# zhoubin-me/agent0

Measured on NVIDIA B200. Metric: replay_sample_target_transitions_per_sec, higher is better.
Workload: dtype u8 frames / f32 targets / f64 n-step returns

## Files before the change

### agent0_b200/_lib.py

```python
import ctypes as C
import os

import torch

_PKG = os.path.dirname(os.path.abspath(__file__))
LIB_PATH = os.environ.get("A0_LIB") or os.path.join(_PKG, "libagent0_b200.so")

A0_SLOTS = 8
A0_REC_META_I32 = 14
A0_MAX_NSTEP = 16
A0_MAX_ACTIONS = 32
A0_MAX_QUANTILES = 256
PTR_FRAMES, PTR_REC_SLOTS, PTR_REC_INFO, PTR_TREE, PTR_MAX_P = range(5)
OPT_PDL = 1
K2B_PLAN_MAX = 1024
K2B_PLAN_BYTES = 90176


def lz4_stride(frame_bytes):
    n = 8 * int(frame_bytes)
    return (n + n // 255 + 20 + 15) // 16 * 16

_vp, _i32, _i64, _f32, _f64 = C.c_void_p, C.c_int32, C.c_int64, C.c_float, C.c_double


class LossCommon(C.Structure):
    _fields_ = [("B", _i32), ("A", _i32), ("action", _vp), ("reward", _vp), ("done", _vp),
                ("weight", _vp), ("gamma_n", _f32), ("alpha", _f32), ("eps", _f32),
                ("loss", _vp), ("prio", _vp), ("max_p", _vp)]


class Plan(C.Structure):
    _fields_ = [("m", _i32), ("n_new", _i32), ("n_marks", _i32), ("new_frame_pos", C.POINTER(_i32)),
                ("rec_meta", C.POINTER(_i32)), ("marks", C.POINTER(_i32))]


class Merge(C.Structure):
    _fields_ = [("n_place", _i64), ("place", C.POINTER(_i64)), ("n_rec", _i64), ("record_map", C.POINTER(_i64)),
                ("n_tail", _i64), ("tails", C.POINTER(_i64)), ("stride_hint", _i64)]


IX_HEAD_Q, IX_TAIL_Q, IX_HEAD_FS, IX_TOP, IX_REC_CAPACITY, IX_FRAME_CAPACITY, IX_NSTEP, IX_AGE_LIMIT, \
    IX_MAX_CHUNK, IX_STATE_WORDS = range(10)
INGEST_FRAMES_ON_DEVICE, INGEST_FRAMES_PINNED, INGEST_COPY_STREAM = 1, 2, 4

SIGNATURES = {
    "a0_version": (_i32, []),
    "a0_last_error": (C.c_char_p, []),
    "a0_set_option": (_i32, [_i32, _i64]),
    "a0_get_option": (_i32, [_i32, C.POINTER(C.c_int64)]),
    "a0_rb_create": (_i32, [C.POINTER(_vp), _i64, _i64, _i32, _i32]),
    "a0_rb_destroy": (_i32, [_vp]),
    "a0_rb_reset": (_i32, [_vp, _vp]),
    "a0_rb_ptr": (_vp, [_vp, _i32]),
    "a0_rb_tree_leaves": (_i64, [_vp]),
    "a0_ix_create": (_i32, [C.POINTER(_vp), _i64, _i64, _i32, _i64]),
    "a0_ix_destroy": (_i32, [_vp]),
    "a0_ix_state": (_i32, [_vp, _vp]),
    "a0_ix_sampleable": (_vp, [_vp]),
    "a0_ix_set_stack": (_i32, [_vp, _i64, _vp]),
    "a0_ix_get_stack": (_i32, [_vp, _i64, _vp]),
    "a0_ix_resolve_shift": (_i32, [_vp, _vp, _vp, _i32, _vp]),
    "a0_ix_plan": (_i32, [_vp, _vp, _vp, _i32, _i32, _vp, _vp, _vp, C.POINTER(Plan)]),
    "a0_dd_create": (_i32, [C.POINTER(_vp), _i32]),
    "a0_dd_destroy": (_i32, [_vp]),
    "a0_dd_resolve": (_i32, [_vp, _vp, _vp, _vp, _i32, _vp, _vp, C.POINTER(_i32)]),
    "a0_ex_create": (_i32, [C.POINTER(_vp), _vp, _vp]),
    "a0_ex_destroy": (_i32, [_vp]),
    "a0_ex_extend": (_i32, [_vp, _vp, _vp, _vp, _vp, _vp, _vp, _i32, _f32, _vp]),
    "a0_ex_extend_v": (_i32, [_vp, _vp, _vp, _vp, _vp, _vp, _vp, _i32, _f32, _vp]),
    "a0_ex_decode": (_i32, [_vp, _vp, _vp, _i32, _vp, _vp, _vp]),
    "a0_ex_resolve": (_i32, [_vp, _vp, _vp, _i32, _vp, _vp, C.POINTER(_i32)]),
    "a0_ex_last_timing": (_i32, [_vp, _vp]),
    "a0_lz4_encode": (_i32, [_vp, _i32, _i32, _vp, _vp, _vp, _vp]),
    "a0_ix_serialize": (_i32, [_vp, _vp, _i64, C.POINTER(_i64)]),
    "a0_ix_deserialize": (_i32, [_vp, _vp, _i64]),
    "a0_ckpt_save": (_i32, [_vp, _vp, _vp, C.c_char_p, _vp, _i64, _vp]),
    "a0_ckpt_load": (_i32, [_vp, _vp, _vp, C.c_char_p, _vp, _i64, C.POINTER(_i64), _vp]),
    "a0_ckpt_last_timing": (_i32, [_vp]),
    "a0_ix_merge": (_i32, [_vp, _i32, _vp, _vp, _vp, _vp, _vp, _vp, _vp, _vp, _vp, _vp, _vp, C.POINTER(Merge)]),
    "a0_ckpt_info": (_i32, [C.c_char_p, _vp, _vp, _i64]),
    "a0_ckpt_merge": (_i32, [_vp, _vp, _vp, _vp, _i32, _vp, _vp, _vp, _vp, _i64, _vp, _vp]),
    "a0_rb_ingest_plan": (_i32, [_vp, C.POINTER(Plan), _vp, _vp, _i32, _f32, _vp]),
    "a0_rb_ingest_steps": (_i32, [_vp, _vp, _vp, _vp, _vp, _i32, _vp, _vp, _vp, _i32, _f32, _vp]),
    "a0_rb_ingest_steps_dyn": (_i32, [_vp, _vp, _vp, _vp, _vp, _i32, _vp, _vp, _vp, _i32, _f32, _f32, _i32, _vp]),
    "a0_rb_append": (_i32, [_vp, _vp, _vp, _i32, _vp, _i32, _vp]),
    "a0_pt_mark": (_i32, [_vp, _vp, _i32, _f32, _vp]),
    "a0_pt_update": (_i32, [_vp, _vp, _vp, _i32, _f32, _f32, _vp]),
    "a0_pt_update_report": (_i32, [_vp, _vp, _vp, _i32, _f32, _f32, _vp, _vp, _vp]),
    "a0_pt_update_overlapped": (_i32, [_vp, _vp, _vp, _i32, _f32, _f32, _vp, _vp, _vp]),
    "a0_pt_update_plan": (_i32, [_vp, _vp, _i32, _vp, _vp]),
    "a0_pt_update_apply": (_i32, [_vp, _vp, _vp, _i32, _f32, _f32, _vp, _vp, _vp, _vp]),
    "a0_host_map": (_i32, [_vp, C.POINTER(_vp)]),
    "a0_pt_set": (_i32, [_vp, _vp, _vp, _i32, _vp]),
    "a0_rb_set_dynamic": (_i32, [_vp, _f32, _f32, _f32, _vp]),
    "a0_pt_sample": (_i32, [_vp, _vp, _i32, _i32, _f32, _f32, _f32, _i32, _vp, _vp, _vp, _vp]),
    "a0_pt_sample_rng": (_i32, [_vp, C.c_uint64, _i64, _i32, _i32, _f32, _f32, _f32, _i32, _vp, _vp, _vp, _vp, _vp]),
    "a0_pt_rng_seek": (_i32, [_vp, C.c_uint64, _vp]),
    "a0_pt_sample_unique": (_i32, [_vp, C.c_uint64, _i64, _i32, _i32, _f32, _f32, _f32, _i32, _vp, _vp, _vp, _vp, _vp]),
    "a0_rb_gather": (_i32, [_vp, _vp, _i32, _i32, _f64, _vp, _vp, _vp, _vp, _vp, _vp, _vp, _i32, _vp]),
    "a0_rb_sample_gather": (_i32, [_vp, _vp, C.c_uint64, _i64, _i32, _i32, _f32, _f32, _f32, _i32, _vp, _vp, _vp, _i32, _f64,
                                   _vp, _vp, _vp, _vp, _vp, _vp, _vp, _vp]),
    "a0_rb_sample_mail": (_i32, [_vp, _vp, C.c_uint64, _i64, _i32, _i32, _f32, _f32, _f32, _i32, _vp, _vp, _vp, _vp]),
    "a0_rb_gather_mail": (_i32, [_vp, _i32, _i32, _i32, _i32, _f64, _vp, _vp, _vp, _vp, _vp, _vp, _vp, _vp]),
    "a0_rb_gather_unpaired": (_i32, [_vp, _i32, _vp, _vp]),
    "a0_rb_check_fault": (_i32, [_vp]),
    "a0_rb_gather_f32": (_i32, [_vp, _vp, _i32, _i32, _f64, _vp, _vp, _i32, _vp, _vp, _vp, _vp, _vp, _vp, _vp]),
    "a0_rb_gather_bf16": (_i32, [_vp, _vp, _i32, _i32, _f64, _vp, _vp, _i32, _vp, _vp, _vp, _vp, _vp, _vp, _vp]),
    "a0_loss_dqn": (_i32, [C.POINTER(LossCommon), _vp, _vp, _vp, _vp, _vp]),
    "a0_loss_mdqn": (_i32, [C.POINTER(LossCommon), _vp, _vp, _vp, _f32, _f32, _vp, _vp]),
    "a0_loss_c51": (_i32, [C.POINTER(LossCommon), _vp, _vp, _vp, _vp, _i32, _f32, _f32, _vp, _vp, _vp]),
    "a0_c51_div_check": (_i32, [_f32, _f32, _i32, _vp, _vp]),
    "a0_loss_quantile": (_i32, [C.POINTER(LossCommon), _i32, _vp, _vp, _vp, _vp, _i32, _i32, _vp,
                                _vp, _vp, _vp, _vp, _vp]),
    "a0_act_epsilon_greedy": (_i32, [_vp, _i32, _i32, _f64, _vp, _vp, _vp, _vp, _vp, _vp, _vp]),
    "a0_u8_to_f32": (_i32, [_vp, _vp, _i64, _i32, _vp]),
}

_lib = None


def load():
    global _lib
    if _lib is not None:
        return _lib
    if not os.path.exists(LIB_PATH):
        raise RuntimeError(
            f"{LIB_PATH} is missing: build it with `python -m agent0_b200.build` "
            "(agent0_b200 has no CPU fallback)")
    lib = C.CDLL(LIB_PATH)
    for name, (res, args) in SIGNATURES.items():
        fn = getattr(lib, name)
        fn.restype, fn.argtypes = res, args
    _lib = lib
    return lib


_pyingest = False


def pyingest():
    global _pyingest
    if _pyingest is False:
        path = os.path.join(_PKG, "_a0_pyingest.so")
        _pyingest = None
        if os.path.exists(path):
            try:
                h = C.PyDLL(path)
                h.a0_py_unpack.restype = _i64
                h.a0_py_unpack.argtypes = [C.py_object, _i64, _vp, _vp, _vp, _vp, _vp, _vp]
                h.a0_py_release.restype = None
                h.a0_py_release.argtypes = [_i64, _vp]
                h.a0_py_buffer_size.restype = _i64
                _pyingest = h
            except OSError:
                _pyingest = None
    return _pyingest


def check(rc, what):
    if rc != 0:
        msg = load().a0_last_error().decode(errors="replace")
        raise RuntimeError(f"{what} failed (code {rc}): {msg}")

# ... 61 lines not shown
```

### agent0_b200/csrc/a0_targets.cu

```cuda
#include <stdlib.h>

#include "a0_common.cuh"
#ifdef A0_TRACE
A0_TRACE_SETTER(a0_trace_set_targets)
#endif

struct A0Common {
  int32_t B, A;
  const int64_t* action;
  const float* reward;
  const float* done;
  const float* weight;
  float gamma_n, alpha, eps;
  float* loss;
  float* prio;
  float* max_p;
};

static inline A0Common a0_unpack(const a0_loss_common_t* c) {
  A0Common k;
  k.B = c->B; k.A = c->A; k.action = c->action; k.reward = c->reward; k.done = c->done;
  k.weight = c->weight; k.gamma_n = c->gamma_n; k.alpha = c->alpha; k.eps = c->eps;
  k.loss = c->loss; k.prio = c->prio; k.max_p = c->max_p;
  return k;
// ... 292 lines not shown
#pragma unroll
  for (int k = 0; k < C51_MAXR; ++k) m[k] = s_m[wid][lane + 32 * k];

  A0_TX(4);
  const float lse = logf(ose);
  float ce = 0.0f, msum = 0.0f;
#pragma unroll
  for (int k = 0; k < C51_MAXR; ++k)
    if (k < R && lane + 32 * k < M) { ce += m[k] * ((l[k] - omx) - lse); msum += m[k]; }
  ce = a0_warp_sum(ce);
  msum = a0_warp_sum(msum);
  A0_TX(5);
  float* grow = grad + (size_t)b * A * M;
  for (int a2 = 0; a2 < A; ++a2) {
    if (a2 == a) continue;
    for (int j = lane; j < M; j += 32) grow[(size_t)a2 * M + j] = 0.0f;
  }
#pragma unroll
  for (int k = 0; k < C51_MAXR; ++k) {
    const int j = lane + 32 * k;
    if (k < R && j < M) {
      const float sm = expf((l[k] - omx) - lse);
      grow[(size_t)a * M + j] = w * (sm * msum - m[k]);
      if (target_prob) target_prob[(size_t)b * M + j] = m[k];
    }
  }
  A0_TX(6);
  if (lane == 0) a0_emit(c, b, -ce);
  A0_TX(7);
#ifdef A0_TRACE
  _t2 = _t2 * 0 + (unsigned long long)_c0;
#endif
  if (threadIdx.x == 0) A0_TEND(4);
}


__device__ __forceinline__ float a0_warp_max_redux(float v) {
  float m;
  asm("redux.sync.max.f32 %0, %1, 0xffffffff;" : "=f"(m) : "f"(v));
  return m;
}

__device__ __forceinline__ float a0_c51_div_delta(float nu, float delta, double rdelta) {
  const double q0 = __dmul_rn((double)nu, rdelta);
  const double rem = __fma_rn(-q0, (double)delta, (double)nu);
  return __double2float_rn(__fma_rn(rem, rdelta, q0));
}

static void a0_c51_delta(float vmin, float vmax, int32_t M, float* delta, double* rdelta) {
  *delta = (vmax - vmin) / (float)(M - 1);
  *rdelta = 1.0 / (double)*delta;
}

template <int WARPS>
__global__ void __launch_bounds__(WARPS * 32)
a0_k4_c51_fast(const A0Common c, const float* __restrict__ logits, const float* __restrict__ tgt_logits,
               const float* __restrict__ qsel, const float* __restrict__ atoms, int32_t M, float vmin, float vmax,
               float delta, double rdelta, float* __restrict__ grad, float* __restrict__ target_prob) {
  __shared__ float s_t[WARPS][4][72];
  A0_T0();
  A0_PDL_PROLOGUE();
  A0_TMID();
#ifdef A0_TRACE
  const long long _c0 = clock64();
#endif
  const int lane = threadIdx.x & 31;
  const int wid = threadIdx.x >> 5;
  const int b = blockIdx.x * WARPS + wid;
  if (b >= c.B) return;
  const int A = c.A;
  const bool in0 = lane < M, in1 = lane + 32 < M;
  float lo_all[C51_SPEC_A][2], tg_all[C51_SPEC_A][2], qs[C51_SPEC_A];
  const float* lrow = logits + (size_t)b * A * M + lane;
  const float* trow = tgt_logits + (size_t)b * A * M + lane;
  const float* qrow = qsel + (size_t)b * A;
#pragma unroll
  for (int a2 = 0; a2 < C51_SPEC_A; ++a2) {
    const bool on = a2 < A;
    lo_all[a2][0] = (on && in0) ? lrow[a2 * M] : -INFINITY;
    lo_all[a2][1] = (on && in1) ? lrow[a2 * M + 32] : -INFINITY;
    tg_all[a2][0] = (on && in0) ? trow[a2 * M] : -INFINITY;
    tg_all[a2][1] = (on && in1) ? trow[a2 * M + 32] : -INFINITY;
    qs[a2] = on ? qrow[a2] : -INFINITY;
  }
  const int a = (int)c.action[b];
  const float r = c.reward[b], d = c.done[b], w = c.weight[b];
  const float z0 = in0 ? atoms[lane] : 0.0f, z1 = in1 ? atoms[lane + 32] : 0.0f;
  float(*terms)[72] = s_t[wid];
#pragma unroll
  for (int t = 0; t < 4; ++t) {
    terms[t][lane] = 0.0f;
    terms[t][lane + 32] = 0.0f;
  }
  const int AM = A * M, r0 = a * M;
  float* gb = grad + (size_t)b * AM;
  for (int e = lane; e < AM; e += 32)
    if (e < r0 || e >= r0 + M) gb[e] = 0.0f;
  int a_star = 0;
  float best = qs[0];
#pragma unroll
  for (int a2 = 1; a2 < C51_SPEC_A; ++a2)
    if (qs[a2] > best) { best = qs[a2]; a_star = a2; }
  float l0 = -INFINITY, l1 = -INFINITY, p0 = -INFINITY, p1 = -INFINITY;
#pragma unroll
  for (int a2 = 0; a2 < C51_SPEC_A; ++a2) {
    if (a2 == a) { l0 = lo_all[a2][0]; l1 = lo_all[a2][1]; }
    if (a2 == a_star) { p0 = tg_all[a2][0]; p1 = tg_all[a2][1]; }
  }
  A0_TX(0);
  const float omx = a0_warp_max_redux(fmaxf(l0, l1)), mx = a0_warp_max_redux(fmaxf(p0, p1));
  A0_TX(1);
  const float eo0 = expf(in0 ? l0 - omx : -INFINITY), eo1 = expf(in1 ? l1 - omx : -INFINITY);
  p0 = expf(in0 ? p0 - mx : -INFINITY);
  p1 = expf(in1 ? p1 - mx : -INFINITY);
  float ose = eo0 + eo1, se = p0 + p1;
  const float gm = __fmul_rn(c.gamma_n, __fsub_rn(1.0f, d));
  const float tz0 = fminf(fmaxf(__fadd_rn(r, __fmul_rn(gm, z0)), vmin), vmax);
  const float tz1 = fminf(fmaxf(__fadd_rn(r, __fmul_rn(gm, z1)), vmin), vmax);
  const float bs0 = a0_c51_div_delta(__fsub_rn(tz0, vmin), delta, rdelta);
  const float bs1 = a0_c51_div_delta(__fsub_rn(tz1, vmin), delta, rdelta);
  const int c0 = max((int)ceilf(bs0) - 1, 0), c1 = max((int)ceilf(bs1) - 1, 0);
  const int k0 = in0 ? c0 : -1, k1 = in1 ? c1 : -1;
  const float fl0 = __fsub_rn((float)(c0 + 1), bs0), fu0 = __fsub_rn(bs0, (float)c0);
  const float fl1 = __fsub_rn((float)(c1 + 1), bs1), fu1 = __fsub_rn(bs1, (float)c1);
  unsigned join0 = 0, join1 = 0;
#pragma unroll
  for (int s = 0; s < 5; ++s) {
    const int q0 = __shfl_up_sync(0xffffffffu, k0, 1 << s), q1 = __shfl_up_sync(0xffffffffu, k1, 1 << s);
    if (lane >= (1 << s) && q0 == k0) join0 |= 1u << s;
    if (lane >= (1 << s) && q1 == k1) join1 |= 1u << s;
  }
  const int n0 = __shfl_down_sync(0xffffffffu, k0, 1), n1 = __shfl_down_sync(0xffffffffu, k1, 1);
  const bool tail0 = k0 >= 0 && (lane == 31 || n0 != k0), tail1 = k1 >= 0 && (lane == 31 || n1 != k1);
#pragma unroll
  for (int o = 16; o > 0; o >>= 1) {
    const float a_ = __shfl_xor_sync(0xffffffffu, ose, o);
    const float b_ = __shfl_xor_sync(0xffffffffu, se, o);
    ose += a_;
    se += b_;
  }
  const float lse = logf(ose);
  const float ls0 = (l0 - omx) - lse, ls1 = (l1 - omx) - lse;
  float sm0 = expf(ls0), sm1 = expf(ls1);
  A0_TX(2);
  float wl0 = 0.0f, wu0 = 0.0f, wl1 = 0.0f, wu1 = 0.0f;
  {
    const float q0 = __fdiv_rn(p0 != 0.0f ? p0 : 1.0f, se), q1 = __fdiv_rn(p1 != 0.0f ? p1 : 1.0f, se);
    const float pj0 = p0 != 0.0f ? q0 : 0.0f, pj1 = p1 != 0.0f ? q1 : 0.0f;
    if (in0) { wl0 = __fmul_rn(pj0, fl0); wu0 = __fmul_rn(pj0, fu0); }
    if (in1) { wl1 = __fmul_rn(pj1, fl1); wu1 = __fmul_rn(pj1, fu1); }
  }
  A0_TX(3);
#pragma unroll
  for (int s = 0; s < 5; ++s) {
    const float a0_ = __shfl_up_sync(0xffffffffu, wl0, 1 << s), b0_ = __shfl_up_sync(0xffffffffu, wu0, 1 << s);
    const float a1_ = __shfl_up_sync(0xffffffffu, wl1, 1 << s), b1_ = __shfl_up_sync(0xffffffffu, wu1, 1 << s);
    if (join0 >> s & 1u) { wl0 = __fadd_rn(wl0, a0_); wu0 = __fadd_rn(wu0, b0_); }
    if (join1 >> s & 1u) { wl1 = __fadd_rn(wl1, a1_); wu1 = __fadd_rn(wu1, b1_); }
  }
  asm volatile("" : "+f"(sm0), "+f"(sm1));
  __syncwarp();
  if (tail0) { terms[0][k0] = wl0; terms[2][k0 + 1] = wu0; }
  if (tail1) { terms[1][k1] = wl1; terms[3][k1 + 1] = wu1; }
  __syncwarp();
  const float m0 = __fadd_rn(__fadd_rn(__fadd_rn(terms[0][lane], terms[1][lane]), terms[2][lane]), terms[3][lane]);
  const float m1 = __fadd_rn(__fadd_rn(__fadd_rn(terms[0][lane + 32], terms[1][lane + 32]), terms[2][lane + 32]),
                             terms[3][lane + 32]);
  A0_TX(4);
  float ce = 0.0f, msum = 0.0f;
  if (in0) { ce += m0 * ls0; msum += m0; }
  if (in1) { ce += m1 * ls1; msum += m1; }
#pragma unroll
  for (int o = 16; o > 0; o >>= 1) {
    const float a_ = __shfl_xor_sync(0xffffffffu, ce, o);
    const float b_ = __shfl_xor_sync(0xffffffffu, msum, o);
    ce += a_;
    msum += b_;
  }
  A0_TX(5);
  if (lane == 0) a0_emit(c, b, -ce);
  const float g0 = w * (sm0 * msum - m0), g1 = w * (sm1 * msum - m1);
  if (in0) gb[r0 + lane] = g0;
  if (in1) gb[r0 + lane + 32] = g1;
  if (target_prob) {
    if (in0) target_prob[(size_t)b * M + lane] = m0;
    if (in1) target_prob[(size_t)b * M + lane + 32] = m1;
  }
  A0_TX(6);
  A0_TX(7);
#ifdef A0_TRACE
  _t2 = _t2 * 0 + (unsigned long long)_c0;
#endif
  if (threadIdx.x == 0) A0_TEND(4);
}

static int g_c51_fast = -1;
static bool a0_option_c51_fast() {
  if (g_c51_fast < 0) {
    const char* e = getenv("A0_C51_FAST");
    g_c51_fast = e ? (atoi(e) != 0) : 1;
  }
  return g_c51_fast != 0;
}
void a0_set_c51_fast(int on) { g_c51_fast = on != 0; }

extern "C" int a0_loss_c51(const a0_loss_common_t* c, const float* logits, const float* tgt_logits,
                           const float* qsel, const float* atoms, int32_t M, float vmin, float vmax, float* grad,
                           float* target_prob, a0_stream_t stream) {
  int rc = a0_check_common(c, "a0_loss_c51");
  if (rc) return rc;
  A0_REQUIRE(logits && tgt_logits && atoms && grad, "a0_loss_c51: NULL tensor");
  A0_REQUIRE(M >= 2 && M <= C51_MAXR * 32, "a0_loss_c51: num_atoms %d outside [2,%d]", M, C51_MAXR * 32);
  A0_REQUIRE(vmax > vmin, "a0_loss_c51: vmax must exceed vmin");
  if (c->B == 0) return A0_OK;
  float delta;
  double rdelta;
  a0_c51_delta(vmin, vmax, M, &delta, &rdelta);
  if (qsel && c->A <= C51_SPEC_A && M <= 64 && delta > 0.0f && delta < INFINITY && a0_option_c51_fast()) {
    static int warps = 0;
    if (!warps) {
      const char* e = getenv("A0_C51_WARPS");
      warps = e ? atoi(e) : C51_FAST_WARPS;
      if (warps != 1 && warps != 2 && warps != 4 && warps != 8 && warps != 16 && warps != 32) warps = C51_FAST_WARPS;
    }
    const unsigned grid = (unsigned)((c->B + warps - 1) / warps);
#define A0_C51_FAST_LAUNCH(W)                                                                                              \
    A0_LAUNCH(a0_k4_c51_fast<W>, grid, W * 32, 0, (cudaStream_t)stream, 1, A0_PDL_K4, a0_unpack(c), logits, tgt_logits, qsel,   \
              atoms, M, vmin, vmax, delta, rdelta, grad, target_prob)
    if (warps == 1) A0_C51_FAST_LAUNCH(1);
    else if (warps == 2) A0_C51_FAST_LAUNCH(2);
    else if (warps == 4) A0_C51_FAST_LAUNCH(4);
    else if (warps == 8) A0_C51_FAST_LAUNCH(8);
    else if (warps == 16) A0_C51_FAST_LAUNCH(16);
    else A0_C51_FAST_LAUNCH(32);
#undef A0_C51_FAST_LAUNCH
    return A0_OK;
  }
  A0_LAUNCH(a0_k4_c51, (unsigned)((c->B + C51_WARPS - 1) / C51_WARPS), C51_WARPS * 32, 0, (cudaStream_t)stream, 1, A0_PDL_K4,
            a0_unpack(c), logits, tgt_logits, qsel, atoms, M, vmin, vmax, grad, target_prob);
  return A0_OK;
}

__global__ void a0_c51_div_check_kernel(uint32_t hi, float delta, double rdelta, unsigned long long* out) {
  unsigned long long bad = 0, first = ~0ull;
  for (unsigned long long u = blockIdx.x * (unsigned long long)blockDim.x + threadIdx.x; u <= hi;
       u += (unsigned long long)gridDim.x * blockDim.x) {
    const float nu = __uint_as_float((uint32_t)u);
    if (__float_as_uint(a0_c51_div_delta(nu, delta, rdelta)) != __float_as_uint(__fdiv_rn(nu, delta))) {
      ++bad;
      first = min(first, u);
    }
  }
  if (bad) {
    atomicAdd(out, bad);
    atomicMin(out + 1, first);
  }
}

extern "C" int a0_c51_div_check(float vmin, float vmax, int32_t M, unsigned long long* out, a0_stream_t stream) {
  A0_REQUIRE(out != nullptr, "a0_c51_div_check: NULL output");
  A0_REQUIRE(M >= 2 && vmax > vmin, "a0_c51_div_check: M %d, vmin %g, vmax %g", M, (double)vmin, (double)vmax);
  float delta;
  double rdelta;
  a0_c51_delta(vmin, vmax, M, &delta, &rdelta);
  A0_REQUIRE(delta > 0.0f && delta < INFINITY, "a0_c51_div_check: delta %g is zero or infinite", (double)delta);
  const float hi = vmax - vmin;
  A0_REQUIRE(hi < INFINITY, "a0_c51_div_check: vmax - vmin overflows");
  uint32_t hb;
  memcpy(&hb, &hi, sizeof(hb));
  a0_c51_div_check_kernel<<<148 * 8, 256, 0, (cudaStream_t)stream>>>(hb, delta, rdelta, out);
  A0_LAUNCH_CHECK();
  return A0_OK;
}

constexpr int QH_SPEC_A = 8;

__device__ __forceinline__ float a0_block_sum(float v, float* red, int nwarps) {
  v = a0_warp_sum(v);
  __syncthreads();
  if ((threadIdx.x & 31) == 0) red[threadIdx.x >> 5] = v;
  __syncthreads();
  float s = 0.0f;
  for (int i = 0; i < nwarps; ++i) s += red[i];
  return s;
}

template <bool SPEC>
__global__ void __launch_bounds__(A0_MAX_QUANTILES)
a0_k4_quantile(const A0Common c, int32_t layout, const float* __restrict__ q, const float* __restrict__ qt,
               const float* __restrict__ taus, const float* __restrict__ qsel, int32_t Ni, int32_t Nj,
               float* __restrict__ grad, const float* __restrict__ q_bar, const float* __restrict__ taus_full,
               float* __restrict__ fraction_loss, float* __restrict__ grad_taus) {
  __shared__ float sT[A0_MAX_QUANTILES];
// ... 592 lines not shown
```

### agent0_b200/hotloop.py

```python
from __future__ import annotations

import ctypes as C

import numpy as np
import torch

from . import _lib

ALGOS = ("dqn", "mdqn", "c51", "qr", "iqn", "fqf")


def wave_plan(L, B, frame_bytes, spec="auto"):
    if not spec or L < 2:
        return None
    if isinstance(spec, str):
        assert spec == "auto", spec
        if B * 16 * frame_bytes >= 10_000_000:
            sizes = [1] * L
        else:
            sizes, w = [1], 1
            while sum(sizes) < L:
                sizes.append(min(w, L - sum(sizes)))
                w *= 2
            if len(sizes) > 1 and sizes[-1] < sizes[-2]:
                tail = sizes.pop()
                sizes[-1] += tail
    else:
        sizes = [int(x) for x in spec]
        assert all(x > 0 for x in sizes) and sum(sizes) == L, "gather_waves must be positive batch counts that sum to learner_steps"
    if len(sizes) < 2:
        return None
    plan, b0 = [], 0
    for n in sizes:
        plan.append((b0, n, b0 * B, n * B))
        b0 += n
    return plan


class ReplayTargetLoop:
    def __init__(self, replay, algo, batch_size, learner_steps, action_dim, outputs, n_step=None, double_q=True,
                 per=None, variant=0, discount=None, alpha=0.5, eps=0.01, c51=(51, -10.0, 10.0), mdqn=(0.03, -1.0),
                 frames=None, rng_seed=None, overlap_sample_gather=None, want_prio=False, early_update=True,
                 gather_waves="auto", pdl_at_joins=True, gather_window="auto", k4_priority=True, waves_when_eager=False,
                 replacement=True):
        assert algo in ALGOS, algo
        self.lib = _lib.load()
        self.rp, self.algo, self.B, self.L, self.A = replay, algo, int(batch_size), int(learner_steps), int(action_dim)
        self.total = T = self.L * self.B
        self.dev = dev = replay.device
        self.variant = int(variant)
        self.replacement = bool(replacement)
        if not self.replacement:
            if overlap_sample_gather:
                raise ValueError("ReplayTargetLoop(replacement=False) gathers with one plain launch: the overlapped / waved "
                                 "sample-gather schedules draw with replacement only")
            if self.B > 1024:
                raise ValueError(f"ReplayTargetLoop(replacement=False) takes batches of at most 1024 records, not {self.B}")
            if rng_seed is None:
                rng_seed = int(torch.randint(-2 ** 63, 2 ** 63 - 1, (1,), dtype=torch.int64).item())
        elif overlap_sample_gather is None:
            overlap_sample_gather = True
        self.overlap_sg = bool(overlap_sample_gather) and int(variant) == 0
        self.early_update = bool(early_update)
        self.rng_seed = None if rng_seed is None else int(rng_seed) & 0xFFFFFFFFFFFFFFFF
        self.n = int(n_step if n_step is not None else replay.n_gather)
        self.gamma = float(discount if discount is not None else replay.gamma)
        self.gamma_n = float(np.float32(self.gamma ** self.n))
        self.per = replay.prioritize if per is None else bool(per)
        self.double_q = bool(double_q)
        self.alpha, self.eps = float(alpha), float(eps)
        self.c51, self.mdqn = c51, mdqn
        e = lambda *s, dt=torch.float32: torch.empty(*s, dtype=dt, device=dev)
        self.u = e(T)
        self.idx = e(T, dt=torch.int64); self.prio = e(T); self.w = e(T)
        self.frames = frames if frames is not None else e(T, 8 * replay.F, dt=torch.uint8)
        self.act = e(T, dt=torch.int64); self.r64 = e(T, dt=torch.float64); self.r32 = e(T)
        self.d8 = e(T, dt=torch.uint8); self.d32 = e(T); self.boot = e(T, dt=torch.int64)
        self.loss = e(T); self.newp = e(T) if want_prio else None
        self.o = outputs
        self.grad = torch.empty_like(self.o["online"])
        self.frac = e(T) if algo == "fqf" else None
        self.gtau = e(T, self.o["taus"].shape[1]) if algo == "fqf" else None
        self.waves = self._wave_plan(gather_waves) if self.overlap_sg else None
        self.pdl_at_joins = bool(pdl_at_joins)
        self.waves_when_eager = bool(waves_when_eager)
        if self.waves:
            self.side = torch.cuda.Stream(device=dev)
            self.fast = torch.cuda.Stream(device=dev, priority=-1) if k4_priority else None
            self.wave_ev = [torch.cuda.Event() for _ in self.waves]
            self._join = {b0: j for j, (b0, _, _, _) in enumerate(self.waves)}
            per_batch = self.B * 16 * replay.F >= 10_000_000
            self.window = (400 if per_batch else 128) if gather_window == "auto" else int(gather_window or 0)
        n_gather = len(self.waves) if self.waves else 1
        self._plan_join = max(self.waves[-1][0] + 1, self.L - 4) if self.waves else self.L
        self._use_plan = self._use_plan_default = self.per and self.early_update and T <= _lib.K2B_PLAN_MAX and self._plan_join < self.L
        if self._use_plan:
            self.plan = torch.empty(_lib.K2B_PLAN_BYTES, dtype=torch.uint8, device=dev)
            self.plan_ev = torch.cuda.Event()
        self.launches_per_step = 1 + n_gather + self.L + (1 if self.per else 0)
        self._k4 = None
        self._k4_all = None
        self.graph = None
        self.report = []
        self._report_dev = []
        self.graphs = []

    def _st(self):
        return _lib.stream_ptr(self.dev)

    def sample(self):
        rp = self.rp
        if not self.replacement:
            _lib.check(self.lib.a0_pt_sample_unique(rp.h, self.rng_seed, -1, self.total, self.B, -1.0, float(rp.beta), 0.0,
                                                    0 if self.per else 1, self.idx.data_ptr(), self.prio.data_ptr(),
                                                    self.w.data_ptr(), None, self._st()), "a0_pt_sample_unique")
            return
        if self.rng_seed is not None:
            _lib.check(self.lib.a0_pt_sample_rng(rp.h, self.rng_seed, -1, self.total, self.B, -1.0, float(rp.beta), 0.0,
                                                 0 if self.per else 1, self.idx.data_ptr(), self.prio.data_ptr(),
                                                 self.w.data_ptr(), None, self._st()), "a0_pt_sample_rng")
            return
        _lib.check(self.lib.a0_pt_sample(rp.h, self.u.data_ptr(), self.total, self.B, -1.0, float(rp.beta), 0.0,
                                         0 if self.per else 1, self.idx.data_ptr(), self.prio.data_ptr(),
                                         self.w.data_ptr(), self._st()), "a0_pt_sample")

    def gather(self, idx_ptr=None, out_ptr=None, count=None, variant=None):
        _lib.check(self.lib.a0_rb_gather(self.rp.h, idx_ptr or self.idx.data_ptr(), count or self.total, self.n, self.gamma,
                                         out_ptr or self.frames.data_ptr(), self.act.data_ptr(), self.r64.data_ptr(),
                                         self.r32.data_ptr(), self.d8.data_ptr(), self.d32.data_ptr(), self.boot.data_ptr(),
                                         self.variant if variant is None else variant, self._st()), "a0_rb_gather")

    def sample_gather(self):
        rp = self.rp
        _lib.check(self.lib.a0_rb_sample_gather(
            rp.h, None if self.rng_seed is not None else self.u.data_ptr(), self.rng_seed or 0, -1, self.total, self.B, -1.0,
            float(rp.beta), 0.0, 0 if self.per else 1, self.idx.data_ptr(), self.prio.data_ptr(), self.w.data_ptr(), self.n,
            self.gamma, self.frames.data_ptr(), self.act.data_ptr(), self.r64.data_ptr(), self.r32.data_ptr(),
            self.d8.data_ptr(), self.d32.data_ptr(), self.boot.data_ptr(), self._st()), "a0_rb_sample_gather")

    def _wave_plan(self, spec):
        return wave_plan(self.L, self.B, self.rp.F, spec)

    def sample_gather_waves(self, plan=False):
        rp, lib = self.rp, self.lib
        main = torch.cuda.current_stream(self.dev)
        self.side.wait_stream(main)
        with torch.cuda.stream(self.side):
            st = self._st()
            _lib.check(lib.a0_rb_sample_mail(rp.h, None if self.rng_seed is not None else self.u.data_ptr(), self.rng_seed or 0, -1,
                                             self.total, self.B, -1.0, float(rp.beta), 0.0, 0 if self.per else 1, self.idx.data_ptr(),
                                             self.prio.data_ptr(), self.w.data_ptr(), st), "a0_rb_sample_mail")
            for j, (_, _, lo, cnt) in enumerate(self.waves):
                _lib.check(lib.a0_rb_gather_mail(rp.h, lo, cnt, self.window, self.n, self.gamma, self.frames.data_ptr(), self.act.data_ptr(),
                                                 self.r64.data_ptr(), self.r32.data_ptr(), self.d8.data_ptr(), self.d32.data_ptr(),
                                                 self.boot.data_ptr(), st), "a0_rb_gather_mail")
                self.wave_ev[j].record(self.side)
            if plan:
                _lib.check(lib.a0_pt_update_plan(rp.h, self.idx.data_ptr(), self.total, self.plan.data_ptr(), st), "a0_pt_update_plan")
                self.plan_ev.record(self.side)

    def _wait_wave(self, j):
        torch.cuda.current_stream(self.dev).wait_event(self.wave_ev[j])

    def _common(self, lo, count):
        s = slice(lo, lo + count)
        p = lambda t: t[s].data_ptr()
        return _lib.LossCommon(B=count, A=self.A, action=p(self.act), reward=p(self.r32), done=p(self.d32), weight=p(self.w),
                               gamma_n=self.gamma_n, alpha=self.alpha, eps=self.eps, loss=p(self.loss), prio=p(self.newp) if self.newp is not None else None,
                               max_p=self.rp.max_p_tensor.data_ptr() if self.per else None), s

    def _bind(self, lo, count):
        lib, o, algo = self.lib, self.o, self.algo
        c, s = self._common(lo, count)
        p = lambda t: t[s].data_ptr()
        qsel = p(o["qsel"]) if (self.double_q or algo in ("iqn", "fqf")) and algo != "mdqn" else None
        if algo == "dqn":
            a = (lib.a0_loss_dqn, (C.byref(c), p(o["online"]), p(o["tgt_next"]), qsel, p(self.grad)))
        elif algo == "mdqn":
            a = (lib.a0_loss_mdqn, (C.byref(c), p(o["online"]), p(o["tgt_next"]), p(o["tgt_cur"]), self.mdqn[0], self.mdqn[1],
                                    p(self.grad)))
        elif algo == "c51":
            M, vmin, vmax = self.c51
            a = (lib.a0_loss_c51, (C.byref(c), p(o["online"]), p(o["tgt_next"]), qsel, o["atoms"].data_ptr(), M, vmin, vmax,
                                   p(self.grad), None))
        elif algo == "qr":
            N = o["online"].shape[2]
            a = (lib.a0_loss_quantile, (C.byref(c), 0, p(o["online"]), p(o["tgt_next"]), None, qsel, o["tgt_next"].shape[2], N,
                                        p(self.grad), None, None, None, None))
        elif algo == "iqn":
            a = (lib.a0_loss_quantile, (C.byref(c), 1, p(o["online"]), p(o["tgt_next"]), p(o["taus"]), qsel,
                                        o["tgt_next"].shape[1], o["online"].shape[1], p(self.grad), None, None, None, None))
        else:
            F_ = o["online"].shape[1]
            a = (lib.a0_loss_quantile, (C.byref(c), 1, p(o["online"]), p(o["tgt_next"]), p(o["taus_hat"]), qsel, F_, F_,
                                        p(self.grad), p(o["q_bar"]), p(o["taus"]), p(self.frac), p(self.gtau)))
        return c, a

    def target_loss(self, k):
        if self._k4 is None:
            self._k4 = [self._bind(k_ * self.B, self.B) for k_ in range(self.L)]
        fn, args = self._k4[k][1]
        rc = fn(*args, self._st())
        if rc:
            _lib.check(rc, "a0_loss_" + self.algo)

    def target_loss_all(self):
        if self._k4_all is None:
            self._k4_all = self._bind(0, self.total)
        fn, args = self._k4_all[1]
        rc = fn(*args, self._st())
        if rc:
            _lib.check(rc, "a0_loss_" + self.algo)

    def bind_report(self, slots=2):
        self.report = [(torch.empty(self.total, dtype=torch.int64).pin_memory(),
                        torch.empty(self.total, dtype=torch.float32).pin_memory()) for _ in range(int(slots))]
        self._report_dev = [(_lib.host_map(i), _lib.host_map(l)) for i, l in self.report]
        return self.report

    def update(self, slot=None, after_k4=False):
        if self.per and self.early_update and after_k4:
            ri, rl = self._report_dev[slot] if slot is not None else (None, None)
            _lib.check(self.lib.a0_pt_update_overlapped(self.rp.h, self.idx.data_ptr(), self.loss.data_ptr(), self.total, self.alpha,
                                                        self.eps, ri, rl, self._st()), "a0_pt_update_overlapped")
            return
        if self.per and slot is not None:
            ri, rl = self._report_dev[slot]
            _lib.check(self.lib.a0_pt_update_report(self.rp.h, self.idx.data_ptr(), self.loss.data_ptr(), self.total, self.alpha,
                                                    self.eps, ri, rl, self._st()), "a0_pt_update_report")
            return
        if self.per:
            _lib.check(self.lib.a0_pt_update(self.rp.h, self.idx.data_ptr(), self.loss.data_ptr(), self.total, self.alpha,
                                             self.eps, self._st()), "a0_pt_update")
        if slot is not None:
            self.report[slot][0].copy_(self.idx, non_blocking=True)
            self.report[slot][1].copy_(self.loss, non_blocking=True)

    def _apply(self, slot=None):
        ri, rl = self._report_dev[slot] if slot is not None else (None, None)
        _lib.check(self.lib.a0_pt_update_apply(self.rp.h, self.idx.data_ptr(), self.loss.data_ptr(), self.total, self.alpha,
                                               self.eps, self.plan.data_ptr(), ri, rl, self._st()), "a0_pt_update_apply")

    def _targets_and_update(self, fused_k4, slot, update=True, planned=False):
        if fused_k4:
            for j in range(len(self.waves)):
                self._wait_wave(j)
            self.target_loss_all()
            if update:
                self.update(slot, after_k4=True)
            return
        for k in range(self.L):
            j = self._join.get(k)
            join_plan = planned and k == self._plan_join
            if join_plan:
                torch.cuda.current_stream(self.dev).wait_event(self.plan_ev)
            if (j is None and not join_plan) or self.pdl_at_joins:
                if j is not None:
                    self._wait_wave(j)
                self.target_loss(k)
            else:
                if j is not None:
                    self._wait_wave(j)
                mask = C.c_int64(0)
                _lib.check(self.lib.a0_get_option(_lib.OPT_PDL, C.byref(mask)), "a0_get_option")
                self.lib.a0_set_option(_lib.OPT_PDL, mask.value & ~1)
                try:
                    self.target_loss(k)
                finally:
                    self.lib.a0_set_option(_lib.OPT_PDL, mask.value)
        if planned:
            self._apply(slot)
        elif update:
            self.update(slot, after_k4=True)

    def step(self, fused_k4=False, slot=None, update=True):
        if self.rng_seed is None:
            self.u.uniform_()
        if self.waves and (self.waves_when_eager or torch.cuda.is_current_stream_capturing()):
            planned = update and self._use_plan and not fused_k4
            self.sample_gather_waves(plan=planned)
            if self.fast is None:
                self._targets_and_update(fused_k4, slot, update, planned)
                return
            main = torch.cuda.current_stream(self.dev)
            self.fast.wait_stream(main)
            with torch.cuda.stream(self.fast):
                self._targets_and_update(fused_k4, slot, update, planned)
            main.wait_stream(self.fast)
            return
        if self.overlap_sg:
            self.sample_gather()
        else:
            self.sample()
            self.gather()
        if fused_k4:
            self.target_loss_all()
        else:
            for k in range(self.L):
                self.target_loss(k)
        if update:
            self.update(slot, after_k4=True)

    def capture(self, warm=3, fused_k4=False):
        self.rp.push_dynamic()
        for _ in range(warm):
            self.step(fused_k4)
        torch.cuda.synchronize(self.dev)
        g = torch.cuda.CUDAGraph()
        with torch.cuda.graph(g):
            self.step(fused_k4)
        self.graph = g
        return g
# ... 80 lines not shown
```

### include/agent0_b200.h

```cpp
#ifndef AGENT0_B200_H
#define AGENT0_B200_H

#include <stddef.h>
#include <stdint.h>

#ifdef __cplusplus
extern "C" {
#endif

typedef struct a0_replay a0_replay_t;
typedef struct a0_index a0_index_t;
typedef void* a0_stream_t;

#define A0_OK 0
#define A0_EINVAL (-1)
#define A0_ENOMEM (-2)
#define A0_EFAULT (-3)
#define A0_STACK 4
#define A0_SLOTS 8
#define A0_MAX_NSTEP 16
#define A0_MAX_ACTIONS 32
#define A0_MAX_QUANTILES 256
#define A0_REC_META_I32 14

// ... 157 lines not shown
                        float* prio_out, float* weight_out, int32_t* stats_out, a0_stream_t stream);

int a0_rb_gather(a0_replay_t* h, const int64_t* idx , int32_t count, int32_t n_step,
                 double gamma, uint8_t* frames_out, int64_t* action_out, double* reward64_out,
                 float* reward32_out, uint8_t* done8_out, float* done32_out, int64_t* boot_out,
                 int32_t variant, a0_stream_t stream);

int a0_rb_sample_gather(a0_replay_t* h, const float* u , uint64_t seed,
                        int64_t call, int32_t total, int32_t batch, float top, float beta,
                        float sum_offset, int32_t uniform, int64_t* idx_out, float* prio_out,
                        float* weight_out, int32_t n_step, double gamma, uint8_t* frames_out,
                        int64_t* action_out, double* reward64_out, float* reward32_out,
                        uint8_t* done8_out, float* done32_out, int64_t* boot_out, a0_stream_t stream);

int a0_rb_sample_mail(a0_replay_t* h, const float* u , uint64_t seed, int64_t call,
                      int32_t total, int32_t batch, float top, float beta, float sum_offset, int32_t uniform,
                      int64_t* idx_out, float* prio_out, float* weight_out, a0_stream_t stream);
int a0_rb_gather_mail(a0_replay_t* h, int32_t lo, int32_t count, int32_t window, int32_t n_step, double gamma,
                      uint8_t* frames_out, int64_t* action_out, double* reward64_out, float* reward32_out,
                      uint8_t* done8_out, float* done32_out, int64_t* boot_out, a0_stream_t stream);

int a0_rb_gather_unpaired(a0_replay_t* h, int32_t count, uint8_t* frames_out, a0_stream_t stream);
int a0_rb_check_fault(a0_replay_t* h);

int a0_rb_gather_f32(a0_replay_t* h, const int64_t* idx , int32_t count, int32_t n_step,
                     double gamma, float* obs_out, float* next_out, int32_t norm_mode,
                     int64_t* action_out, double* reward64_out, float* reward32_out,
                     uint8_t* done8_out, float* done32_out, int64_t* boot_out, a0_stream_t stream);
int a0_rb_gather_bf16(a0_replay_t* h, const int64_t* idx , int32_t count, int32_t n_step,
                      double gamma, uint16_t* obs_out, uint16_t* next_out, int32_t norm_mode,
                      int64_t* action_out, double* reward64_out, float* reward32_out,
                      uint8_t* done8_out, float* done32_out, int64_t* boot_out, a0_stream_t stream);

typedef struct {
  int32_t B, A;
  const int64_t* action;
  const float* reward;
  const float* done;
  const float* weight;
  float gamma_n;
  float alpha, eps;
  float* loss;
  float* prio;
  float* max_p;
} a0_loss_common_t;

int a0_loss_dqn(const a0_loss_common_t* c, const float* q, const float* qt_next, const float* qsel,
                float* grad, a0_stream_t stream);
int a0_loss_mdqn(const a0_loss_common_t* c, const float* q, const float* qt_next,
                 const float* qt_cur, float tau, float lo, float* grad, a0_stream_t stream);
int a0_loss_c51(const a0_loss_common_t* c, const float* logits, const float* tgt_logits,
                const float* qsel, const float* atoms, int32_t M, float vmin, float vmax,
                float* grad, float* target_prob, a0_stream_t stream);
int a0_c51_div_check(float vmin, float vmax, int32_t M, unsigned long long* out, a0_stream_t stream);
int a0_loss_quantile(const a0_loss_common_t* c, int32_t layout, const float* q, const float* qt,
                     const float* taus, const float* qsel, int32_t Ni, int32_t Nj, float* grad,
                     const float* q_bar, const float* taus_full, float* fraction_loss,
                     float* grad_taus, a0_stream_t stream);

int a0_act_epsilon_greedy(const float* q , int32_t E, int32_t A, double epsilon,
                          const double* u , const int64_t* action_random ,
                          int64_t* action_out, float* qmax_out, float* scratch, float* qmax_mean,
                          a0_stream_t stream);
int a0_u8_to_f32(const uint8_t* in , float* out , int64_t count, int32_t norm_mode,
                 a0_stream_t stream);

#ifdef __cplusplus
}
#endif
#endif
```

Measured before the change: 11.49 million.

## Compute C51 projection geometry before PDL wait on non-join links

Adds an EARLY template variant of the fast C51 target kernel. It reads the batch-side inputs (action, reward, done, weight), zeroes the gradient rows and computes the projection bins and warp join masks before the programmatic-dependent-launch wait. After the wait it loads only the selected action's online logits. The hot loop uses this variant for links that are not wave or plan joins, so this prologue work overlaps the tail of the previous kernel. The risk is correctness: the early reads and gradient writes must not depend on or race with the preceding kernel's outputs.

```diff
diff --git a/agent0_b200/_lib.py b/agent0_b200/_lib.py
--- a/agent0_b200/_lib.py
+++ b/agent0_b200/_lib.py
@@ -15,6 +15,7 @@
 OPT_PDL = 1
 K2B_PLAN_MAX = 1024
 K2B_PLAN_BYTES = 90176
+C51_EARLY = 1
 
 
 def lz4_stride(frame_bytes):
@@ -110,6 +111,7 @@
     "a0_loss_dqn": (_i32, [C.POINTER(LossCommon), _vp, _vp, _vp, _vp, _vp]),
     "a0_loss_mdqn": (_i32, [C.POINTER(LossCommon), _vp, _vp, _vp, _f32, _f32, _vp, _vp]),
     "a0_loss_c51": (_i32, [C.POINTER(LossCommon), _vp, _vp, _vp, _vp, _i32, _f32, _f32, _vp, _vp, _vp]),
+    "a0_loss_c51_linked": (_i32, [C.POINTER(LossCommon), _vp, _vp, _vp, _vp, _i32, _f32, _f32, _vp, _vp, _i32, _vp]),
     "a0_c51_div_check": (_i32, [_f32, _f32, _i32, _vp, _vp]),
     "a0_loss_quantile": (_i32, [C.POINTER(LossCommon), _i32, _vp, _vp, _vp, _vp, _i32, _i32, _vp,
                                 _vp, _vp, _vp, _vp, _vp]),
diff --git a/agent0_b200/csrc/a0_targets.cu b/agent0_b200/csrc/a0_targets.cu
--- a/agent0_b200/csrc/a0_targets.cu
+++ b/agent0_b200/csrc/a0_targets.cu
@@ -368,17 +368,22 @@
   *rdelta = 1.0 / (double)*delta;
 }
 
-template <int WARPS>
+template <int WARPS, bool EARLY>
 __global__ void __launch_bounds__(WARPS * 32)
 a0_k4_c51_fast(const A0Common c, const float* __restrict__ logits, const float* __restrict__ tgt_logits,
                const float* __restrict__ qsel, const float* __restrict__ atoms, int32_t M, float vmin, float vmax,
                float delta, double rdelta, float* __restrict__ grad, float* __restrict__ target_prob) {
   __shared__ float s_t[WARPS][4][72];
   A0_T0();
-  A0_PDL_PROLOGUE();
-  A0_TMID();
 #ifdef A0_TRACE
-  const long long _c0 = clock64();
+  _tx[7] = (unsigned long long)clock64();
+#endif
+  if (!EARLY) {
+    A0_PDL_PROLOGUE();
+    A0_TMID();
+  }
+#ifdef A0_TRACE
+  long long _c0 = clock64();
 #endif
   const int lane = threadIdx.x & 31;
   const int wid = threadIdx.x >> 5;
@@ -386,41 +391,89 @@
   if (b >= c.B) return;
   const int A = c.A;
   const bool in0 = lane < M, in1 = lane + 32 < M;
+  float(*terms)[72] = s_t[wid];
+  int a, r0;
+  float r, d, w, z0, z1;
+  float* gb;
+  auto batch_side = [&] {
+    a = (int)c.action[b];
+    r = c.reward[b], d = c.done[b], w = c.weight[b];
+    z0 = in0 ? atoms[lane] : 0.0f, z1 = in1 ? atoms[lane + 32] : 0.0f;
+#pragma unroll
+    for (int t = 0; t < 4; ++t) {
+      terms[t][lane] = 0.0f;
+      terms[t][lane + 32] = 0.0f;
+    }
+    const int AM = A * M;
+    r0 = a * M;
+    gb = grad + (size_t)b * AM;
+    for (int e = lane; e < AM; e += 32)
+      if (e < r0 || e >= r0 + M) gb[e] = 0.0f;
+  };
+  int k0, k1;
+  float fl0, fu0, fl1, fu1;
+  unsigned join0 = 0, join1 = 0;
+  unsigned tail0, tail1;
+  auto geometry = [&] {
+    const float gm = __fmul_rn(c.gamma_n, __fsub_rn(1.0f, d));
+    const float tz0 = fminf(fmaxf(__fadd_rn(r, __fmul_rn(gm, z0)), vmin), vmax);
+    const float tz1 = fminf(fmaxf(__fadd_rn(r, __fmul_rn(gm, z1)), vmin), vmax);
+    const float bs0 = a0_c51_div_delta(__fsub_rn(tz0, vmin), delta, rdelta);
+    const float bs1 = a0_c51_div_delta(__fsub_rn(tz1, vmin), delta, rdelta);
+    const int c0 = max((int)ceilf(bs0) - 1, 0), c1 = max((int)ceilf(bs1) - 1, 0);
+    k0 = in0 ? c0 : -1, k1 = in1 ? c1 : -1;
+    fl0 = __fsub_rn((float)(c0 + 1), bs0), fu0 = __fsub_rn(bs0, (float)c0);
+    fl1 = __fsub_rn((float)(c1 + 1), bs1), fu1 = __fsub_rn(bs1, (float)c1);
+#pragma unroll
+    for (int s = 0; s < 5; ++s) {
+      const int q0 = __shfl_up_sync(0xffffffffu, k0, 1 << s), q1 = __shfl_up_sync(0xffffffffu, k1, 1 << s);
+      if (lane >= (1 << s) && q0 == k0) join0 |= 1u << s;
+      if (lane >= (1 << s) && q1 == k1) join1 |= 1u << s;
+    }
+    const int n0 = __shfl_down_sync(0xffffffffu, k0, 1), n1 = __shfl_down_sync(0xffffffffu, k1, 1);
+    tail0 = k0 >= 0 && (lane == 31 || n0 != k0), tail1 = k1 >= 0 && (lane == 31 || n1 != k1);
+  };
+  if (EARLY) {
+    batch_side();
+    geometry();
+    asm volatile("" : "+r"(k0), "+r"(k1), "+f"(fl0), "+f"(fu0), "+f"(fl1), "+f"(fu1), "+r"(join0), "+r"(join1),
+                 "+r"(tail0), "+r"(tail1), "+r"(a), "+f"(w));
+    A0_PDL_PROLOGUE();
+    A0_TMID();
+#ifdef A0_TRACE
+    _c0 = clock64();
+#endif
+  }
   float lo_all[C51_SPEC_A][2], tg_all[C51_SPEC_A][2], qs[C51_SPEC_A];
+  float l0 = -INFINITY, l1 = -INFINITY, p0 = -INFINITY, p1 = -INFINITY;
   const float* lrow = logits + (size_t)b * A * M + lane;
   const float* trow = tgt_logits + (size_t)b * A * M + lane;
   const float* qrow = qsel + (size_t)b * A;
+  if (EARLY) {
+    const bool on = a >= 0 && a < A;
+    l0 = (on && in0) ? lrow[a * M] : -INFINITY;
+    l1 = (on && in1) ? lrow[a * M + 32] : -INFINITY;
+  }
 #pragma unroll
   for (int a2 = 0; a2 < C51_SPEC_A; ++a2) {
     const bool on = a2 < A;
-    lo_all[a2][0] = (on && in0) ? lrow[a2 * M] : -INFINITY;
-    lo_all[a2][1] = (on && in1) ? lrow[a2 * M + 32] : -INFINITY;
+    if (!EARLY) {
+      lo_all[a2][0] = (on && in0) ? lrow[a2 * M] : -INFINITY;
+      lo_all[a2][1] = (on && in1) ? lrow[a2 * M + 32] : -INFINITY;
+    }
     tg_all[a2][0] = (on && in0) ? trow[a2 * M] : -INFINITY;
     tg_all[a2][1] = (on && in1) ? trow[a2 * M + 32] : -INFINITY;
     qs[a2] = on ? qrow[a2] : -INFINITY;
   }
-  const int a = (int)c.action[b];
-  const float r = c.reward[b], d = c.done[b], w = c.weight[b];
-  const float z0 = in0 ? atoms[lane] : 0.0f, z1 = in1 ? atoms[lane + 32] : 0.0f;
-  float(*terms)[72] = s_t[wid];
-#pragma unroll
-  for (int t = 0; t < 4; ++t) {
-    terms[t][lane] = 0.0f;
-    terms[t][lane + 32] = 0.0f;
-  }
-  const int AM = A * M, r0 = a * M;
-  float* gb = grad + (size_t)b * AM;
-  for (int e = lane; e < AM; e += 32)
-    if (e < r0 || e >= r0 + M) gb[e] = 0.0f;
+  if (!EARLY) batch_side();
   int a_star = 0;
   float best = qs[0];
 #pragma unroll
   for (int a2 = 1; a2 < C51_SPEC_A; ++a2)
     if (qs[a2] > best) { best = qs[a2]; a_star = a2; }
-  float l0 = -INFINITY, l1 = -INFINITY, p0 = -INFINITY, p1 = -INFINITY;
 #pragma unroll
   for (int a2 = 0; a2 < C51_SPEC_A; ++a2) {
-    if (a2 == a) { l0 = lo_all[a2][0]; l1 = lo_all[a2][1]; }
+    if (!EARLY && a2 == a) { l0 = lo_all[a2][0]; l1 = lo_all[a2][1]; }
     if (a2 == a_star) { p0 = tg_all[a2][0]; p1 = tg_all[a2][1]; }
   }
   A0_TX(0);
@@ -430,24 +483,7 @@
   p0 = expf(in0 ? p0 - mx : -INFINITY);
   p1 = expf(in1 ? p1 - mx : -INFINITY);
   float ose = eo0 + eo1, se = p0 + p1;
-  const float gm = __fmul_rn(c.gamma_n, __fsub_rn(1.0f, d));
-  const float tz0 = fminf(fmaxf(__fadd_rn(r, __fmul_rn(gm, z0)), vmin), vmax);
-  const float tz1 = fminf(fmaxf(__fadd_rn(r, __fmul_rn(gm, z1)), vmin), vmax);
-  const float bs0 = a0_c51_div_delta(__fsub_rn(tz0, vmin), delta, rdelta);
-  const float bs1 = a0_c51_div_delta(__fsub_rn(tz1, vmin), delta, rdelta);
-  const int c0 = max((int)ceilf(bs0) - 1, 0), c1 = max((int)ceilf(bs1) - 1, 0);
-  const int k0 = in0 ? c0 : -1, k1 = in1 ? c1 : -1;
-  const float fl0 = __fsub_rn((float)(c0 + 1), bs0), fu0 = __fsub_rn(bs0, (float)c0);
-  const float fl1 = __fsub_rn((float)(c1 + 1), bs1), fu1 = __fsub_rn(bs1, (float)c1);
-  unsigned join0 = 0, join1 = 0;
-#pragma unroll
-  for (int s = 0; s < 5; ++s) {
-    const int q0 = __shfl_up_sync(0xffffffffu, k0, 1 << s), q1 = __shfl_up_sync(0xffffffffu, k1, 1 << s);
-    if (lane >= (1 << s) && q0 == k0) join0 |= 1u << s;
-    if (lane >= (1 << s) && q1 == k1) join1 |= 1u << s;
-  }
-  const int n0 = __shfl_down_sync(0xffffffffu, k0, 1), n1 = __shfl_down_sync(0xffffffffu, k1, 1);
-  const bool tail0 = k0 >= 0 && (lane == 31 || n0 != k0), tail1 = k1 >= 0 && (lane == 31 || n1 != k1);
+  if (!EARLY) geometry();
 #pragma unroll
   for (int o = 16; o > 0; o >>= 1) {
     const float a_ = __shfl_xor_sync(0xffffffffu, ose, o);
@@ -503,7 +539,6 @@
     if (in1) target_prob[(size_t)b * M + lane + 32] = m1;
   }
   A0_TX(6);
-  A0_TX(7);
 #ifdef A0_TRACE
   _t2 = _t2 * 0 + (unsigned long long)_c0;
 #endif
@@ -520,14 +555,14 @@
 }
 void a0_set_c51_fast(int on) { g_c51_fast = on != 0; }
 
-extern "C" int a0_loss_c51(const a0_loss_common_t* c, const float* logits, const float* tgt_logits,
-                           const float* qsel, const float* atoms, int32_t M, float vmin, float vmax, float* grad,
-                           float* target_prob, a0_stream_t stream) {
-  int rc = a0_check_common(c, "a0_loss_c51");
+static int a0_loss_c51_launch(const char* fn, const a0_loss_common_t* c, const float* logits, const float* tgt_logits,
+                              const float* qsel, const float* atoms, int32_t M, float vmin, float vmax, float* grad,
+                              float* target_prob, bool early, a0_stream_t stream) {
+  int rc = a0_check_common(c, fn);
   if (rc) return rc;
-  A0_REQUIRE(logits && tgt_logits && atoms && grad, "a0_loss_c51: NULL tensor");
-  A0_REQUIRE(M >= 2 && M <= C51_MAXR * 32, "a0_loss_c51: num_atoms %d outside [2,%d]", M, C51_MAXR * 32);
-  A0_REQUIRE(vmax > vmin, "a0_loss_c51: vmax must exceed vmin");
+  A0_REQUIRE(logits && tgt_logits && atoms && grad, "%s: NULL tensor", fn);
+  A0_REQUIRE(M >= 2 && M <= C51_MAXR * 32, "%s: num_atoms %d outside [2,%d]", fn, M, C51_MAXR * 32);
+  A0_REQUIRE(vmax > vmin, "%s: vmax must exceed vmin", fn);
   if (c->B == 0) return A0_OK;
   float delta;
   double rdelta;
@@ -541,20 +576,39 @@
     }
     const unsigned grid = (unsigned)((c->B + warps - 1) / warps);
 #define A0_C51_FAST_LAUNCH(W)                                                                                              \
-    A0_LAUNCH(a0_k4_c51_fast<W>, grid, W * 32, 0, (cudaStream_t)stream, 1, A0_PDL_K4, a0_unpack(c), logits, tgt_logits, qsel,   \
-              atoms, M, vmin, vmax, delta, rdelta, grad, target_prob)
-    if (warps == 1) A0_C51_FAST_LAUNCH(1);
-    else if (warps == 2) A0_C51_FAST_LAUNCH(2);
-    else if (warps == 4) A0_C51_FAST_LAUNCH(4);
-    else if (warps == 8) A0_C51_FAST_LAUNCH(8);
-    else if (warps == 16) A0_C51_FAST_LAUNCH(16);
-    else A0_C51_FAST_LAUNCH(32);
+    if (early)                                                                                                             \
+      A0_LAUNCH(a0_k4_c51_fast<W, true>, grid, W * 32, 0, (cudaStream_t)stream, 1, A0_PDL_K4, a0_unpack(c), logits,         \
+                tgt_logits, qsel, atoms, M, vmin, vmax, delta, rdelta, grad, target_prob);                                 \
+    else                                                                                                                   \
+      A0_LAUNCH(a0_k4_c51_fast<W, false>, grid, W * 32, 0, (cudaStream_t)stream, 1, A0_PDL_K4, a0_unpack(c), logits,        \
+                tgt_logits, qsel, atoms, M, vmin, vmax, delta, rdelta, grad, target_prob)
+    if (warps == 1) { A0_C51_FAST_LAUNCH(1); }
+    else if (warps == 2) { A0_C51_FAST_LAUNCH(2); }
+    else if (warps == 4) { A0_C51_FAST_LAUNCH(4); }
+    else if (warps == 8) { A0_C51_FAST_LAUNCH(8); }
+    else if (warps == 16) { A0_C51_FAST_LAUNCH(16); }
+    else { A0_C51_FAST_LAUNCH(32); }
 #undef A0_C51_FAST_LAUNCH
     return A0_OK;
   }
   A0_LAUNCH(a0_k4_c51, (unsigned)((c->B + C51_WARPS - 1) / C51_WARPS), C51_WARPS * 32, 0, (cudaStream_t)stream, 1, A0_PDL_K4,
             a0_unpack(c), logits, tgt_logits, qsel, atoms, M, vmin, vmax, grad, target_prob);
   return A0_OK;
+}
+
+extern "C" int a0_loss_c51(const a0_loss_common_t* c, const float* logits, const float* tgt_logits,
+                           const float* qsel, const float* atoms, int32_t M, float vmin, float vmax, float* grad,
+                           float* target_prob, a0_stream_t stream) {
+  return a0_loss_c51_launch("a0_loss_c51", c, logits, tgt_logits, qsel, atoms, M, vmin, vmax, grad, target_prob, false,
+                            stream);
+}
+
+extern "C" int a0_loss_c51_linked(const a0_loss_common_t* c, const float* logits, const float* tgt_logits,
+                                  const float* qsel, const float* atoms, int32_t M, float vmin, float vmax, float* grad,
+                                  float* target_prob, int32_t flags, a0_stream_t stream) {
+  A0_REQUIRE((flags & ~A0_C51_EARLY) == 0, "a0_loss_c51_linked: unknown flags 0x%x", (unsigned)flags);
+  return a0_loss_c51_launch("a0_loss_c51_linked", c, logits, tgt_logits, qsel, atoms, M, vmin, vmax, grad, target_prob,
+                            (flags & A0_C51_EARLY) != 0, stream);
 }
 
 __global__ void a0_c51_div_check_kernel(uint32_t hi, float delta, double rdelta, unsigned long long* out) {
diff --git a/agent0_b200/hotloop.py b/agent0_b200/hotloop.py
--- a/agent0_b200/hotloop.py
+++ b/agent0_b200/hotloop.py
@@ -35,6 +35,15 @@
         plan.append((b0, n, b0 * B, n * B))
         b0 += n
     return plan
+
+
+def early_links(L, waves, plan_join=None):
+    if not waves:
+        return frozenset()
+    joins = {b0 for b0, _, _, _ in waves}
+    if plan_join is not None:
+        joins.add(plan_join)
+    return frozenset(k for k in range(L) if k not in joins)
 
 
 class ReplayTargetLoop:
@@ -98,7 +107,7 @@
             self.plan = torch.empty(_lib.K2B_PLAN_BYTES, dtype=torch.uint8, device=dev)
             self.plan_ev = torch.cuda.Event()
         self.launches_per_step = 1 + n_gather + self.L + (1 if self.per else 0)
-        self._k4 = None
+        self._k4 = self._k4_early = None
         self._k4_all = None
         self.graph = None
         self.report = []
@@ -169,7 +178,7 @@
                                gamma_n=self.gamma_n, alpha=self.alpha, eps=self.eps, loss=p(self.loss), prio=p(self.newp) if self.newp is not None else None,
                                max_p=self.rp.max_p_tensor.data_ptr() if self.per else None), s
 
-    def _bind(self, lo, count):
+    def _bind(self, lo, count, early=False):
         lib, o, algo = self.lib, self.o, self.algo
         c, s = self._common(lo, count)
         p = lambda t: t[s].data_ptr()
@@ -181,8 +190,12 @@
                                     p(self.grad)))
         elif algo == "c51":
             M, vmin, vmax = self.c51
-            a = (lib.a0_loss_c51, (C.byref(c), p(o["online"]), p(o["tgt_next"]), qsel, o["atoms"].data_ptr(), M, vmin, vmax,
-                                   p(self.grad), None))
+            if early:
+                a = (lib.a0_loss_c51_linked, (C.byref(c), p(o["online"]), p(o["tgt_next"]), qsel, o["atoms"].data_ptr(), M, vmin,
+                                              vmax, p(self.grad), None, _lib.C51_EARLY))
+            else:
+                a = (lib.a0_loss_c51, (C.byref(c), p(o["online"]), p(o["tgt_next"]), qsel, o["atoms"].data_ptr(), M, vmin, vmax,
+                                       p(self.grad), None))
         elif algo == "qr":
             N = o["online"].shape[2]
             a = (lib.a0_loss_quantile, (C.byref(c), 0, p(o["online"]), p(o["tgt_next"]), None, qsel, o["tgt_next"].shape[2], N,
@@ -196,10 +209,11 @@
                                         p(self.grad), p(o["q_bar"]), p(o["taus"]), p(self.frac), p(self.gtau)))
         return c, a
 
-    def target_loss(self, k):
+    def target_loss(self, k, early=False):
         if self._k4 is None:
             self._k4 = [self._bind(k_ * self.B, self.B) for k_ in range(self.L)]
-        fn, args = self._k4[k][1]
+            self._k4_early = [self._bind(k_ * self.B, self.B, early=True) for k_ in range(self.L)] if self.algo == "c51" else None
+        fn, args = (self._k4_early if early and self._k4_early else self._k4)[k][1]
         rc = fn(*args, self._st())
         if rc:
             _lib.check(rc, "a0_loss_" + self.algo)
@@ -249,6 +263,7 @@
             if update:
                 self.update(slot, after_k4=True)
             return
+        early = early_links(self.L, self.waves, self._plan_join if planned else None)
         for k in range(self.L):
             j = self._join.get(k)
             join_plan = planned and k == self._plan_join
@@ -257,7 +272,7 @@
             if (j is None and not join_plan) or self.pdl_at_joins:
                 if j is not None:
                     self._wait_wave(j)
-                self.target_loss(k)
+                self.target_loss(k, early=k in early)
             else:
                 if j is not None:
                     self._wait_wave(j)
diff --git a/include/agent0_b200.h b/include/agent0_b200.h
--- a/include/agent0_b200.h
+++ b/include/agent0_b200.h
@@ -233,6 +233,10 @@
 int a0_loss_c51(const a0_loss_common_t* c, const float* logits, const float* tgt_logits,
                 const float* qsel, const float* atoms, int32_t M, float vmin, float vmax,
                 float* grad, float* target_prob, a0_stream_t stream);
+#define A0_C51_EARLY 1
+int a0_loss_c51_linked(const a0_loss_common_t* c, const float* logits, const float* tgt_logits,
+                       const float* qsel, const float* atoms, int32_t M, float vmin, float vmax,
+                       float* grad, float* target_prob, int32_t flags, a0_stream_t stream);
 int a0_c51_div_check(float vmin, float vmax, int32_t M, unsigned long long* out, a0_stream_t stream);
 int a0_loss_quantile(const a0_loss_common_t* c, int32_t layout, const float* q, const float* qt,
                      const float* taus, const float* qsel, int32_t Ni, int32_t Nj, float* grad,
```

Result: faster. 11.97 million (median of 6 runs) (+4.1%).
